# TAMUparametric/PPOPT

Hardware: NVIDIA B200
Metric: candidate active sets/sec (higher is better)
Workload: dtype f64

## Files before the change

### include/ppgpu.h

```cpp
#ifndef PPGPU_H
#define PPGPU_H

#include <stddef.h>
#include <stdint.h>

#ifdef __cplusplus
extern "C" {
#endif

typedef struct ppgpu_program ppgpu_program;
typedef void* ppgpu_stream;

typedef struct {
    int32_t n;
    int32_t t;
    int32_t m;
    int32_t q;
    int32_t n_eq;
    int32_t is_qp;
} ppgpu_dims;

typedef struct {
    int32_t words;
    int32_t n_ineq;
    int32_t region_rows;
    int32_t use_gram;
    int32_t max_depth;
    int32_t sm_count;
    int32_t lp_columns;
    int32_t reserved;
} ppgpu_info;

#define PPGPU_NUM_COUNTERS 24

const char* ppgpu_last_error(void);
int ppgpu_version(void);

int ppgpu_program_create(const ppgpu_dims* dims, const double* h_A, const double* h_b, const double* h_F,
                         const double* h_A_t, const double* h_b_t, const double* h_Q, const double* h_c,
                         const double* h_H, int device, ppgpu_program** out);
int ppgpu_program_destroy(ppgpu_program* prog);
int ppgpu_program_info(const ppgpu_program* prog, ppgpu_info* out);

#define PPGPU_OPT_K2W_MIN 0
int ppgpu_set_option(ppgpu_program* prog, int32_t option, int64_t value);

int ppgpu_root_level(ppgpu_program* prog, uint64_t* d_masks, int64_t* h_count, ppgpu_stream stream);

int ppgpu_level_eval(ppgpu_program* prog, const uint64_t* d_masks, int64_t n, int32_t k_act, uint8_t* d_status,
                     int32_t stages, ppgpu_stream stream);

#define PPGPU_WITNESS_SLOTS 2
int ppgpu_level_eval_w(ppgpu_program* prog, const uint64_t* d_masks, int64_t n, int32_t k_act, uint8_t* d_status,
                       int32_t stages, uint64_t* d_witness, const uint64_t* d_parent_feas, int64_t parent_nf,
                       const void* d_parent_ws, const uint64_t* d_parent_wit, ppgpu_stream stream);

size_t ppgpu_scan_workspace_bytes(int64_t n);
size_t ppgpu_select_workspace_bytes(int64_t n);
int ppgpu_level_select(ppgpu_program* prog, const uint8_t* d_status, int64_t n, uint8_t bits, uint8_t value,
                       int64_t* d_idx_out, int64_t* h_count, void* d_ws, size_t ws_bytes, ppgpu_stream stream);

int ppgpu_regions_emit(ppgpu_program* prog, const uint64_t* d_masks, const int64_t* d_sel, int64_t n_sel,
                       int32_t k_act, double* d_laws, double* d_rows, int32_t* d_flags, double* d_info,
                       uint8_t* d_status, ppgpu_stream stream);

int ppgpu_children_count(ppgpu_program* prog, const uint64_t* d_masks, const int64_t* d_feas_idx, int64_t nf,
                         int32_t k_act, uint64_t* d_feas_masks, uint64_t* d_survive, int64_t* d_offsets,
                         int64_t* h_total, void* d_ws, size_t ws_bytes, ppgpu_stream stream);
int ppgpu_children_prepare(ppgpu_program* prog, const uint64_t* d_masks, const int64_t* d_feas_idx, int64_t nf,
                           uint64_t* d_feas_masks, void* d_ws, size_t ws_bytes, ppgpu_stream stream);
int ppgpu_children_count_range(ppgpu_program* prog, const uint64_t* d_feas_masks, int64_t nf, int32_t k_act,
                               uint64_t* d_survive, int64_t* d_counts, int64_t p_lo, int64_t p_hi, void* d_ws,
                               size_t ws_bytes, ppgpu_stream stream);
int ppgpu_children_scan(ppgpu_program* prog, int64_t* d_counts_to_offsets, int64_t nf, int64_t* h_total, void* d_ws,
                        size_t ws_bytes, ppgpu_stream stream);
int ppgpu_children_write(ppgpu_program* prog, const uint64_t* d_feas_masks, const uint64_t* d_survive,
                         const int64_t* d_offsets, int64_t nf, uint64_t* d_children, ppgpu_stream stream);
// ... 42 lines not shown
```

### ppopt_b200/_lib.py

```python
import ctypes
import os

_HERE = os.path.dirname(os.path.abspath(__file__))
LIB_PATH = os.path.join(_HERE, 'libppgpu.so')

NUM_COUNTERS = 24
NUM_FAMILIES = 10
FAMILY_NAMES = ('k1_rank', 'k2_feas_lp', 'k34_kkt_cheb', 'k5_emit', 'k6_count', 'k6_write', 'select', 'k2a_relax', 'k2w_walk', 'inherit')
COUNTER_NAMES = ('k1_candidates', 'k2_lps', 'k2_pivots', 'k2_work', 'k4_lps', 'k4_pivots', 'k4_work', 'k5_lps',
                 'k5_pivots', 'k5_work', 'numeric', 'border', 'k6_lookups', 'k2a_tried', 'k2a_certified', 'k2a_steps', 'k2a_work',
                 'k2w_certified', 'k2w_pivots', 'k2w_work', 'k2w_giveup', 'inherited', 'inherit_lookups')

ST_RANK, ST_FEAS, ST_OPT, ST_REGION, ST_BORDER, ST_NUMERIC, ST_THIN = 1, 2, 4, 8, 16, 32, 64
OPT_K2W_MIN = 0
TREE_OPT_INHERIT = 0
WITNESS_SLOTS = 2


class Dims(ctypes.Structure):
    _fields_ = [(k, ctypes.c_int32) for k in ('n', 't', 'm', 'q', 'n_eq', 'is_qp')]


class Info(ctypes.Structure):
    _fields_ = [(k, ctypes.c_int32) for k in
                ('words', 'n_ineq', 'region_rows', 'use_gram', 'max_depth', 'sm_count', 'lp_columns', 'reserved')]


_vp, _i32, _i64, _u8, _sz = ctypes.c_void_p, ctypes.c_int32, ctypes.c_int64, ctypes.c_uint8, ctypes.c_size_t
SYMBOLS = {
    'ppgpu_last_error': (ctypes.c_char_p, []),
    'ppgpu_version': (ctypes.c_int, []),
    'ppgpu_program_create': (ctypes.c_int, [ctypes.POINTER(Dims)] + [_vp] * 8 + [ctypes.c_int, ctypes.POINTER(_vp)]),
    'ppgpu_program_destroy': (ctypes.c_int, [_vp]),
    'ppgpu_program_info': (ctypes.c_int, [_vp, ctypes.POINTER(Info)]),
    'ppgpu_set_option': (ctypes.c_int, [_vp, _i32, _i64]),
    'ppgpu_root_level': (ctypes.c_int, [_vp, _vp, ctypes.POINTER(_i64), _vp]),
    'ppgpu_level_eval': (ctypes.c_int, [_vp, _vp, _i64, _i32, _vp, _i32, _vp]),
    'ppgpu_level_eval_w': (ctypes.c_int, [_vp, _vp, _i64, _i32, _vp, _i32, _vp, _vp, _i64, _vp, _vp, _vp]),
    'ppgpu_scan_workspace_bytes': (_sz, [_i64]),
    'ppgpu_select_workspace_bytes': (_sz, [_i64]),
    'ppgpu_level_select': (ctypes.c_int, [_vp, _vp, _i64, _u8, _u8, _vp, ctypes.POINTER(_i64), _vp, _sz, _vp]),
    'ppgpu_regions_emit': (ctypes.c_int, [_vp, _vp, _vp, _i64, _i32, _vp, _vp, _vp, _vp, _vp, _vp]),
    'ppgpu_children_count': (ctypes.c_int, [_vp, _vp, _vp, _i64, _i32, _vp, _vp, _vp, ctypes.POINTER(_i64), _vp, _sz, _vp]),
    'ppgpu_children_prepare': (ctypes.c_int, [_vp, _vp, _vp, _i64, _vp, _vp, _sz, _vp]),
    'ppgpu_children_count_range': (ctypes.c_int, [_vp, _vp, _i64, _i32, _vp, _vp, _i64, _i64, _vp, _sz, _vp]),
    'ppgpu_children_scan': (ctypes.c_int, [_vp, _vp, _i64, ctypes.POINTER(_i64), _vp, _sz, _vp]),
    'ppgpu_children_write': (ctypes.c_int, [_vp, _vp, _vp, _vp, _i64, _vp, _vp]),
# ... 41 lines not shown
```

### ppopt_b200/csrc/api.cu

```cuda
#include <cstdio>
#include <cstdlib>
#include <cstring>
#include <mutex>
#include <string>
#include <vector>

#include "../../include/ppgpu.h"
#include "common.cuh"
#include "host_math.hpp"
#include "launch.h"

using namespace ppgpu;

static thread_local std::string g_err;

struct ppgpu_program {
    ReducedProgram host;
    DevProgram dev;
    int device = 0;
    int sm_count = 0;
    std::vector<void*> allocs;
    unsigned long long* d_counters = nullptr;
    unsigned long long* d_queue = nullptr;
    int queue_slot = 0;
    long long launches = 0;
    bool profiling = false;
    struct Span { int family; cudaEvent_t a, b; };
    std::vector<Span> spans;
    std::vector<cudaEvent_t> event_pool;
    long long warm_cap = 0;
    double* d_warm_resid = nullptr;
    long long* d_warm_idx = nullptr;
    unsigned long long* d_warm_count = nullptr;
    int* d_k2w_order = nullptr;
    size_t k2w_order_cap = 0;
    long long k2w_min = 100000;
    double prof_ms[PPGPU_NUM_FAMILIES] = {0};
    long long prof_launches[PPGPU_NUM_FAMILIES] = {0};
};

struct ProfScope {
    ppgpu_program* p; cudaStream_t st; int family; cudaEvent_t a = nullptr, b = nullptr;
    static cudaEvent_t get(ppgpu_program* p) {
        if (!p->event_pool.empty()) { cudaEvent_t e = p->event_pool.back(); p->event_pool.pop_back(); return e; }
        cudaEvent_t e; cudaEventCreate(&e); return e;
    }
    ProfScope(ppgpu_program* p_, cudaStream_t st_, int fam) : p(p_), st(st_), family(fam) {
        if (p->profiling) { a = get(p); b = get(p); cudaEventRecord(a, st); }
    }
    ~ProfScope() {
        if (a) { cudaEventRecord(b, st); p->spans.push_back({family, a, b}); }
    }
};

static const int QUEUE_SLOTS = 64;
extern "C" { static void warm_release(ppgpu_program* p); }

static int fail(const char* where, cudaError_t e) {
    g_err = std::string(where) + ": " + cudaGetErrorString(e);
    return -1;
}
static int fail_msg(const std::string& m) { g_err = m; return -2; }

template <class T>
static cudaError_t upload(ppgpu_program* p, const std::vector<T>& v, const T** out) {
    void* d = nullptr;
    const size_t bytes = v.size() * sizeof(T) + 1024;
    cudaError_t e = cudaMalloc(&d, bytes);
    if (e != cudaSuccess) return e;
// ... 67 lines not shown
            (e = upload(p, R.X0t, &D.X0t)) != cudaSuccess || (e = upload(p, R.Q2, &D.Q2)) != cudaSuccess) {
            ppgpu_program_destroy(p);
            return fail("upload LP start dictionary", e);
        }
    }
    void* dc = nullptr;
    if ((e = cudaMalloc(&dc, (CNT_COUNT + QUEUE_SLOTS) * sizeof(unsigned long long))) != cudaSuccess) {
        ppgpu_program_destroy(p);
        return fail("cudaMalloc counters", e);
    }
    p->allocs.push_back(dc);
    cudaMemset(dc, 0, (CNT_COUNT + QUEUE_SLOTS) * sizeof(unsigned long long));
    p->d_counters = (unsigned long long*)dc;
    p->d_queue = p->d_counters + CNT_COUNT;
    *out = p;
    return 0;
}

int ppgpu_program_destroy(ppgpu_program* p) {
    if (!p) return 0;
    for (void* d : p->allocs) cudaFree(d);
    if (p->d_k2w_order) cudaFree(p->d_k2w_order);
    warm_release(p);
    for (auto& s : p->spans) { cudaEventDestroy(s.a); cudaEventDestroy(s.b); }
    for (cudaEvent_t e : p->event_pool) cudaEventDestroy(e);
    delete p;
    return 0;
}

int ppgpu_set_option(ppgpu_program* p, int32_t option, int64_t value) {
    if (!p) return fail_msg("null argument");
    switch (option) {
        case PPGPU_OPT_K2W_MIN: p->k2w_min = value; return 0;
        default: return fail_msg("unknown option");
    }
}

int ppgpu_program_info(const ppgpu_program* p, ppgpu_info* o) {
    if (!p || !o) return fail_msg("null argument");
    const ReducedProgram& R = p->host;
    o->words = R.W; o->n_ineq = R.mi; o->region_rows = R.R0; o->use_gram = R.use_gram;
    o->max_depth = (R.n > R.t ? R.n : R.t) - R.ne;
    o->sm_count = p->sm_count;
    o->lp_columns = k2_pad_columns(R.nfree + 2);
    o->reserved = R.wk_ok;
    return 0;
}

int ppgpu_root_level(ppgpu_program* p, uint64_t* d_masks, int64_t* h_count, ppgpu_stream stream) {
    if (!p || !h_count) return fail_msg("null argument");
    long long cnt = 0;
    cudaError_t e = root_level(p->dev, d_masks, &cnt, (cudaStream_t)stream);
    if (e != cudaSuccess) return fail("root_level", e);
    p->launches += cnt > 0;
    *h_count = cnt;
    return 0;
}

static long long level_chunk() {
    static const long long c = getenv("PPGPU_CHUNK") ? atoll(getenv("PPGPU_CHUNK")) : (1ll << 22);
    return c < 1024 ? 1024 : c;
}
static long long walk_chunk() {
    static const long long c = getenv("PPGPU_WALK_CHUNK") ? atoll(getenv("PPGPU_WALK_CHUNK")) : (1ll << 27);
    return c < 1024 ? 1024 : c;
}
// ... 58 lines not shown
    cudaError_t e;
    if (stages & 1) {
        ProfScope ps(p, st, 0);
        const long long piece = 1ll << 22;
        for (long long off = 0; off < n; off += piece) {
            const long long nn = n - off < piece ? n - off : piece;
            e = launch_k1(p->dev, d_masks + (size_t)off * p->dev.W, nn, k_act, d_status + off, p->d_counters, p->sm_count, st);
            if (e != cudaSuccess) return fail("K1 rank", e);
            if (k_act >= 1 && k_act <= 8) p->launches++;
            p->launches++;
            if (k_act >= 2 && k_act <= p->dev.np) p->launches++;
        }
    }
    if ((stages & 2) && !(stages & 8) && wio.parent_feas && wio.parent_wit && wio.parent_ws && wio.parent_nf > 0) {
        ProfScope ps(p, st, 9);
        e = launch_inherit(p->dev, d_masks, n, d_status, wio.out, wio.parent_feas, wio.parent_nf, wio.parent_ws,
                           wio.parent_wit, p->d_counters, st);
        if (e != cudaSuccess) return fail("witness inheritance", e);
        p->launches++;
    }
    static const int warm_on = getenv("PPGPU_WARM") ? atoi(getenv("PPGPU_WARM")) : 1;
    p->dev.warm_count = nullptr; p->dev.warm_resid = nullptr; p->dev.warm_idx = nullptr; p->dev.warm_cap = 0;
    if ((stages & 2) && !(stages & 8) && k_act >= 1 && p->k2w_min >= 0 && n >= p->k2w_min) {
        ProfScope ps(p, st, 8);
        bool handled = false;
        const size_t want = k2w_order_scratch_ints(walk_chunk());
        if (want > p->k2w_order_cap) {
            if ((e = cudaStreamSynchronize(st)) != cudaSuccess) return fail("K2w order scratch", e);
            if (p->d_k2w_order) cudaFree(p->d_k2w_order);
            p->d_k2w_order = nullptr; p->k2w_order_cap = 0;
            if ((e = cudaMalloc((void**)&p->d_k2w_order, want * sizeof(int))) != cudaSuccess) return fail("K2w order scratch", e);
            p->k2w_order_cap = want;
        }
        e = launch_k2w(p->dev, d_masks, n, k_act, d_status, next_queue(p, st), p->d_counters, p->sm_count, st, &handled, wio.out, p->d_k2w_order);
        if (e != cudaSuccess) return fail("K2w vertex walk", e);
        if (handled) p->launches += (n > 128ll * 8 * p->sm_count) ? 4 : 1;
    }
    if ((stages & 2) && !(stages & 8)) {
        ProfScope ps(p, st, 7);
        static const int iters = getenv("PPGPU_K2A_ITERS") ? atoi(getenv("PPGPU_K2A_ITERS")) : 96;
        if (iters > 0 && k_act >= 0) {
            if (warm_on) {
                const bool walked = k_act >= 1 && p->dev.wk_ok && p->k2w_min >= 0 && n >= p->k2w_min;
                const long long cap = n < 4096 ? n : 4096 + n / (walked ? 64 : 8);
                if ((e = ensure_warm(p, cap, st)) != cudaSuccess) return fail("warm-start buffers", e);
                p->dev.warm_count = p->d_warm_count; p->dev.warm_resid = p->d_warm_resid;
                p->dev.warm_idx = p->d_warm_idx; p->dev.warm_cap = cap;
                cudaMemsetAsync(p->d_warm_count, 0, sizeof(unsigned long long), st);
            }
            e = launch_k2a(p->dev, d_masks, n, k_act, d_status, next_queue(p, st), p->d_counters, iters,
                           p->sm_count, st);
            if (e != cudaSuccess) return fail("K2a relaxation", e);
            p->launches++;
        }
    }
    if (stages & 2) {
        ProfScope ps(p, st, 1);
        e = launch_k2(p->dev, d_masks, n, d_status, next_queue(p, st), p->d_counters, p->sm_count, st);
        if (e != cudaSuccess) return fail("K2 feasibility", e);
        p->launches++;
        if (p->dev.warm_count) {
            if ((e = launch_clear_bits(d_status, n, PPG_ST_PRE, st)) != cudaSuccess) return fail("status clean-up", e);
            p->launches++;
        }
    }
    if (stages & 4) {
        ProfScope ps(p, st, 2);
// ... 412 lines not shown
```

### ppopt_b200/csrc/common.cuh

```cuda
#pragma once
#include <cuda_runtime.h>
#include <stdint.h>

#include "tolerances.h"

namespace ppgpu {

struct DevProgram {
    int n, t, m, q, ne, is_qp;
    int mi, np, W, R0, nfree, use_gram;
    int dc0;
    const double* At;
    const double* C1;
    const double* T0;
    const double* Gam;
    const double* G;
    const double* V;
    const double* th_lo; const double* th_hi;
    const double* A; const double* b; const double* F;
    const double* A_t; const double* b_t;
    const double* Q; const double* c; const double* H;
    const double* Xp;
    const double* K;
    const double* Pm;
    double* warm_resid;
    long long* warm_idx;
    unsigned long long* warm_count;
    long long warm_cap;
    int wk_ok, wk_nb, wk_ld;
    const double* wk_D0;
    const int* wk_bvar;
    const int* wk_nvar;
    int lp_ok, lp_ld;
    const double* lp_D0;
    const int* lp_bvar;
    const int* lp_nvar;
    const double* lp_obj;
    const double* X0t;
    const double* Q2;
};

enum Counter {
    CNT_K1_CAND = 0,
    CNT_K2_LPS, CNT_K2_PIVOTS, CNT_K2_WORK,
    CNT_K4_LPS, CNT_K4_PIVOTS, CNT_K4_WORK,
    CNT_K5_LPS, CNT_K5_PIVOTS, CNT_K5_WORK,
    CNT_NUMERIC, CNT_BORDER, CNT_K6_LOOKUPS,
    CNT_K2A_TRIED, CNT_K2A_CERTIFIED, CNT_K2A_STEPS,
    CNT_K2A_WORK,
    CNT_K2W_CERTIFIED, CNT_K2W_PIVOTS, CNT_K2W_WORK,
    CNT_K2W_GIVEUP,
    CNT_INHERITED, CNT_INHERIT_LOOKUPS,
    CNT_COUNT = 24
};

__device__ __forceinline__ bool mask_test(const uint64_t* m, int i) { return (m[i >> 6] >> (i & 63)) & 1ull; }

__device__ __forceinline__ int mask_popc(const uint64_t* m, int W) {
    int c = 0;
    for (int w = 0; w < W; ++w) c += __popcll(m[w]);
    return c;
}

__device__ __forceinline__ int mask_nth(const uint64_t* m, int W, int j) {
    for (int w = 0; w < W; ++w) {
        const uint64_t x = m[w];
        const int c = __popcll(x);
        if (j < c) {
            const unsigned lo = (unsigned)x, hi = (unsigned)(x >> 32);
            const int cl = __popc(lo);
            if (j < cl) return w * 64 + (int)__fns(lo, 0, j + 1);
            return w * 64 + 32 + (int)__fns(hi, 0, j - cl + 1);
        }
        j -= c;
    }
    return -1;
}

__device__ __forceinline__ int mask_rank(const uint64_t* m, int i) {
    int c = 0;
    const int w = i >> 6;
    for (int k = 0; k < w; ++k) c += __popcll(m[k]);
    const int b = i & 63;
    if (b) c += __popcll(m[w] & ((1ull << b) - 1ull));
    return c;
}
// ... 20 lines not shown
```

### ppopt_b200/csrc/k2w_walk.cu

```cuda
#include "common.cuh"
#include "launch.h"
#include "lp_core.cuh"

#include <cstdlib>

namespace ppgpu {

constexpr int K2W_MAXFIX = 30;
constexpr int K2W_DRIVE_CAP = 400;
constexpr int K2W_RESET = 3000;
constexpr double K2W_PIV_MIN = 1e-7;
constexpr double K2W_NEG_OK = 1e-8;

struct K2wCtx {
    double* D;
    double* prow;
    int* bvar;
    int* nvar;
    int* where;
    uint64_t* orig;
    uint64_t* todo;
    int* rowstart;
    uint64_t* nbm;
    int* fixrow;
    uint64_t* witness;
    int nb, nf, ld, lds, R0, W4, Wm;
};

__device__ __forceinline__ int k2w_top_bit(const uint64_t* m, int W, int* second) {
    int hi1 = -1, hi2 = -1;
    for (int w = W - 1; w >= 0 && hi2 < 0; --w) {
        uint64_t x = m[w];
        while (x && hi2 < 0) {
            const int t = w * 64 + 63 - __clzll((long long)x);
            x &= ~(1ull << (t & 63));
            if (hi1 < 0) hi1 = t; else hi2 = t;
        }
    }
    *second = hi2;
    return hi1;
}

__device__ __forceinline__ int k2w_nth(const uint64_t (&m)[4], int j) {
#pragma unroll
    for (int w = 0; w < 4; ++w) {
// ... 10 lines not shown

__device__ __forceinline__ double k2w_rcp(double x) {
    double r;
    asm("rcp.approx.ftz.f64 %0, %1;" : "=d"(r) : "d"(x));
    r = r * fma(-x, r, 2.0);
    return r * fma(-x, r, 2.0);
}

__device__ __forceinline__ void k2w_swap_labels(const K2wCtx& c, int l, int j) {
    const int rl = c.bvar[l], rn = c.nvar[j];
    c.bvar[l] = rn; c.nvar[j] = rl;
    c.where[rn] = l; c.where[rl] = ~j;
    c.nbm[rn >> 6] &= ~(1ull << (rn & 63));
    c.nbm[rl >> 6] |= 1ull << (rl & 63);
}

__device__ __forceinline__ void k2w_reload_labels(const DevProgram& P, const K2wCtx& c, int lane) {
    for (int w = lane; w < c.W4; w += 32) c.nbm[w] = 0ull;
    __syncwarp();
    for (int i = lane; i < c.nb; i += 32) { const int v = __ldg(P.wk_bvar + i); c.bvar[i] = v; c.where[v] = i; }
    for (int j = lane; j < c.nf; j += 32) {
        const int v = __ldg(P.wk_nvar + j);
        c.nvar[j] = v; c.where[v] = ~j;
        atomicOr(reinterpret_cast<unsigned long long*>(c.nbm + (v >> 6)), 1ull << (v & 63));
    }
    __syncwarp();
}

template <int RPL_, int LD_ = 0>
struct K2wSmemDict {
    static constexpr int RPL = RPL_;
    static constexpr bool IN_SMEM = true;
    static constexpr int SMEM_ROW0 = 0;
    __device__ __forceinline__ void reload(const DevProgram& P, const K2wCtx& c, int lane) {
        for (int e = lane; e < c.nb * c.ld; e += 32) {
            const int r = e / c.ld, k = e - r * c.ld;
            c.D[(size_t)r * c.lds + k] = __ldg(P.wk_D0 + e);
        }
        k2w_reload_labels(P, c, lane);
    }
    __device__ __forceinline__ void target_scan(const K2wCtx& c, int wi, uint64_t fm, int lane, double& bi, double& wbest, int& j) {
        const int lds = LD_ > 0 ? LD_ : c.lds;
        const double* Di = c.D + (size_t)wi * lds;
        bi = Di[0];
        const bool degen = bi <= 1e-11;
        double best = 0.0; int bj = 0x7fffffff;
        for (int jj = lane; jj < c.nf; jj += 32) {
            if ((fm >> jj) & 1ull) continue;
            double x = Di[1 + jj];
            if (degen) x = fabs(x);
            if (x > best) { best = x; bj = jj; }
        }
        wbest = warp_max_nonneg(best);
        j = __reduce_min_sync(PPG_FULL, best == wbest ? bj : 0x7fffffff);
    }
    __device__ __forceinline__ void column(const K2wCtx& c, int j, int lane, double (&col)[RPL], double (&beta)[RPL]) {
#pragma unroll
        for (int rr = 0; rr < RPL; ++rr) {
            const int r = lane + 32 * rr;
            const int lds = LD_ > 0 ? LD_ : c.lds;
            col[rr] = r < c.nb ? c.D[(size_t)r * lds + 1 + j] : 0.0;
            beta[rr] = r < c.nb ? c.D[(size_t)r * lds] : 0.0;
        }
    }
    __device__ __forceinline__ bool pivot(const K2wCtx& c, int l, int j, int lane) {
        const int cj = 1 + j, lds = LD_ > 0 ? LD_ : c.lds, ld = LD_ > 0 ? LD_ : c.ld, nb = c.nb;
// ... 52 lines not shown
#pragma unroll
                    for (int g = 0; g < G; ++g) x[rr][g] = (k0 + g < ld) ? Dr[rr][k0 + g] : 0.0;
#pragma unroll
                for (int rr = 0; rr < RPL; ++rr)
#pragma unroll
                    for (int g = 0; g < G; ++g) x[rr][g] = fma(-colr[rr], qk[g], x[rr][g]);
#pragma unroll
                for (int rr = 0; rr < RPL; ++rr)
                    if (colr[rr] != 0.0) {
#pragma unroll
                        for (int g = 0; g < G; ++g)
                            if (k0 + g < ld) Dr[rr][k0 + g] = x[rr][g];
                    }
            }
        }
        bool ok = okb;
#pragma unroll
        for (int rr = 0; rr < RPL; ++rr) {
            const int r = lane + 32 * rr;
            if (r < nb && r != l) {
                if (colr[rr] != 0.0) Dr[rr][cj] = -colr[rr] * inv;
                if constexpr (LD_ == 0) ok = ok && Dr[rr][0] >= -K2W_NEG_OK;
            }
        }
        __syncwarp();
        for (int k = lane; k < ld; k += 32) Dl[k] = (k == cj) ? inv : q[k];
        if (lane == 0) k2w_swap_labels(c, l, j);
        ok = __all_sync(PPG_FULL, ok);
        __syncwarp();
        return ok;
    }
};

template <int RPL_, int LD>
struct K2wHybridDict {
    static constexpr int RPL = RPL_;
    static constexpr bool IN_SMEM = true;
    static constexpr int SMEM_ROW0 = 32;
    double T0[LD];
    __device__ __forceinline__ void reload(const DevProgram& P, const K2wCtx& c, int lane) {
#pragma unroll
        for (int k = 0; k < LD; ++k) T0[k] = lane < c.nb ? __ldg(P.wk_D0 + (size_t)lane * LD + k) : 0.0;
        for (int e = lane + 32 * LD; e < c.nb * LD; e += 32) c.D[e - 32 * LD] = __ldg(P.wk_D0 + e);
        k2w_reload_labels(P, c, lane);
    }
    __device__ __forceinline__ void target_scan(const K2wCtx& c, int wi, uint64_t fm, int lane, double& bi, double& wbest, int& j) {
        if (wi < 32) {
            const double b0 = T0[0];
            const bool degen = b0 <= 1e-11;
            double best = 0.0; int bj = 0x7fffffff;
#pragma unroll
            for (int k = 1; k < LD; ++k) {
                double x = T0[k];
                if (degen) x = fabs(x);
                if (!((fm >> (k - 1)) & 1ull) && x > best) { best = x; bj = k - 1; }
            }
            bi = shfl_d(b0, wi);
            wbest = shfl_d(best, wi);
            j = __shfl_sync(PPG_FULL, bj, wi);
        } else {
            const double* Di = c.D + (size_t)(wi - 32) * LD;
            bi = Di[0];
            const bool degen = bi <= 1e-11;
            double best = 0.0; int bj = 0x7fffffff;
            for (int jj = lane; jj < c.nf; jj += 32) {
                if ((fm >> jj) & 1ull) continue;
                double x = Di[1 + jj];
                if (degen) x = fabs(x);
                if (x > best) { best = x; bj = jj; }
            }
            wbest = warp_max_nonneg(best);
// ... 67 lines not shown
                for (int rr = 1; rr < RPL; ++rr) {
                    const int r = lane + 32 * rr;
                    okb = okb && (r >= nb || r == l || x[rr][0] >= -K2W_NEG_OK);
                }
            }
#pragma unroll
            for (int rr = 1; rr < RPL; ++rr)
                if (colr[rr] != 0.0) {
#pragma unroll
                    for (int g = 0; g < GN; ++g) Dr[rr][k0 + g] = x[rr][g];
                }
        });
        reg_set<LD>(T0, cj, own ? inv : -colr[0] * inv);
#pragma unroll
        for (int rr = 1; rr < RPL; ++rr) {
            const int r = lane + 32 * rr;
            if (r < nb && r != l && colr[rr] != 0.0) Dr[rr][cj] = -colr[rr] * inv;
        }
        __syncwarp();
        if (!l_in_regs)
            for (int k = lane; k < LD; k += 32) Dl[k] = (k == cj) ? inv : q[k];
        if (lane == 0) k2w_swap_labels(c, l, j);
        const bool ok = __all_sync(PPG_FULL, okb);
        __syncwarp();
        return ok;
    }
};

template <int RPL_, int DC>
struct K2wRegDict {
    static constexpr int RPL = RPL_;
    static constexpr bool IN_SMEM = false;
    static constexpr int SMEM_ROW0 = 0;
    double T[RPL][DC];
    __device__ __forceinline__ void reload(const DevProgram& P, const K2wCtx& c, int lane) {
        static_for<RPL>([&](auto RR) {
            constexpr int rr = decltype(RR)::value;
            const int r = lane + 32 * rr;
#pragma unroll
            for (int k = 0; k < DC; ++k) T[rr][k] = r < c.nb ? __ldg(P.wk_D0 + (size_t)r * DC + k) : 0.0;
        });
        k2w_reload_labels(P, c, lane);
    }
    __device__ __forceinline__ void target_scan(const K2wCtx& c, int wi, uint64_t fm, int lane, double& bi, double& wbest, int& j) {
        const int slot = wi >> 5, owner = wi & 31;
        double b0 = 0.0, best = 0.0; int bj = 0x7fffffff;
        static_for<RPL>([&](auto RR) {
            constexpr int rr = decltype(RR)::value;
            if (rr == slot) {
                b0 = T[rr][0];
                const bool degen = b0 <= 1e-11;
#pragma unroll
                for (int k = 1; k < DC; ++k) {
                    double x = T[rr][k];
                    if (degen) x = fabs(x);
                    if (!((fm >> (k - 1)) & 1ull) && x > best) { best = x; bj = k - 1; }
                }
            }
        });
        bi = shfl_d(b0, owner);
        wbest = shfl_d(best, owner);
        j = __shfl_sync(PPG_FULL, bj, owner);
    }
    __device__ __forceinline__ void column(const K2wCtx& c, int j, int lane, double (&col)[RPL], double (&beta)[RPL]) {
        static_for<RPL>([&](auto RR) {
            constexpr int rr = decltype(RR)::value;
// ... 155 lines not shown
                    *cw &= ~rb;
                    k2w_certify(c, status, seg_base, y, r);
                    ++got;
                }
            }
        }
        __syncwarp();
    }
    return got;
}

template <class Dict>
__host__ __device__ constexpr size_t k2w_dict_smem_bytes(int nb, int lds) {
    if constexpr (!Dict::IN_SMEM) return 0;
    else return (size_t)(nb > Dict::SMEM_ROW0 ? nb - Dict::SMEM_ROW0 : 0) * lds * 8;
}

template <class Dict>
__global__ void __launch_bounds__(256, 1)
k2w_walk_kernel(DevProgram P, const uint64_t* __restrict__ masks, long long n, int k_act, uint8_t* __restrict__ status,
                unsigned long long* __restrict__ queue, unsigned long long* __restrict__ counters, int chunk,
                int walker_bytes, int lds, int W4, int group_items, int split_len, uint64_t* __restrict__ witness,
                const int* __restrict__ order, long long items) {
    extern __shared__ unsigned char k2w_smem[];
    const int warp = threadIdx.x >> 5, lane = threadIdx.x & 31;
    constexpr int RPL = Dict::RPL;
    Dict dict;
    K2wCtx c;
    c.nb = P.wk_nb; c.nf = P.nfree; c.ld = P.wk_ld; c.lds = lds; c.R0 = P.R0; c.W4 = W4;
    c.witness = witness; c.Wm = P.W;
    {
        unsigned char* base = k2w_smem + (size_t)warp * walker_bytes;
        c.D = reinterpret_cast<double*>(base); base += k2w_dict_smem_bytes<Dict>(c.nb, lds);
        c.prow = reinterpret_cast<double*>(base); base += (size_t)lds * 8;
        c.orig = reinterpret_cast<uint64_t*>(base); base += (size_t)c.R0 * W4 * 8;
        c.todo = reinterpret_cast<uint64_t*>(base); base += (size_t)c.R0 * W4 * 8;
        c.nbm = reinterpret_cast<uint64_t*>(base); base += (size_t)W4 * 8;
        c.bvar = reinterpret_cast<int*>(base); base += (size_t)c.nb * 4;
        c.nvar = reinterpret_cast<int*>(base); base += (size_t)c.nf * 4;
        c.where = reinterpret_cast<int*>(base); base += (size_t)c.R0 * 4;
        c.rowstart = reinterpret_cast<int*>(base); base += (size_t)c.R0 * 4;
        c.fixrow = reinterpret_cast<int*>(base);
    }
    const int W = P.W, R0 = P.R0, nb = c.nb, nf = c.nf;
    const int p = k_act >= 2 ? k_act - 2 : 0;
    unsigned long long n_piv = 0, n_give = 0;
    int n_cert = 0;
    auto split = [&](long long q, uint64_t (&pf)[4], int& a, int& b) {
#pragma unroll
        for (int w = 0; w < 4; ++w) pf[w] = w < W ? masks[q * W + w] : 0ull;
        b = k2w_top_bit(pf, W, &a);
        if (k_act < 2) a = b;
        pf[b >> 6] &= ~(1ull << (b & 63));
        if (k_act >= 2) pf[a >> 6] &= ~(1ull << (a & 63));
    };
    auto seg_end = [&](long long from, long long limit, const uint64_t (&pf0)[4], int a_ref) -> long long {
        for (long long q0 = from; q0 < limit; q0 += 32) {
            const long long q = q0 + lane;
            bool same = true;
            if (q < limit) {
                uint64_t m[4]; int a1, b1;
                split(q, m, a1, b1);
                same = m[0] == pf0[0] && m[1] == pf0[1] && m[2] == pf0[2] && m[3] == pf0[3] && (a_ref < 0 || a1 == a_ref);
            }
            const unsigned diff = __ballot_sync(PPG_FULL, !same);
            if (diff) return q0 + __ffs((int)diff) - 1;
        }
        return limit;
    };
    for (;;) {
        unsigned long long v = 0;
        if (lane == 0) {
            v = atomicAdd(queue, 1ull);
            if (v < (unsigned long long)items && order) v = (unsigned long long)order[v];
        }
        const long long item = (long long)__shfl_sync(PPG_FULL, v, 0);
        if (item >= items) break;
        const long long c0 = item * chunk;
        const long long c1 = (c0 + chunk < n) ? c0 + chunk : n;
// ... 23 lines not shown
            int any = 0;
            for (long long q0 = i; q0 < s1; q0 += 32) {
                const long long q = q0 + lane;
                int a1 = -1, b1 = -1;
                bool open = false;
                if (q < s1) {
                    uint64_t m[4];
                    split(q, m, a1, b1);
                    const uint8_t sb = status[q];
                    open = (sb & PPG_ST_RANK) && !(sb & PPG_ST_FEAS);
                    atomicOr(reinterpret_cast<unsigned long long*>(c.orig + (size_t)a1 * W4 + (b1 >> 6)), 1ull << (b1 & 63));
                    if ((sb & PPG_ST_RANK) && a1 != b1)
                        atomicOr(reinterpret_cast<unsigned long long*>(c.orig + (size_t)b1 * W4 + (a1 >> 6)), 1ull << (a1 & 63));
                    if (open) {
                        atomicOr(reinterpret_cast<unsigned long long*>(c.todo + (size_t)a1 * W4 + (b1 >> 6)), 1ull << (b1 & 63));
                        if (a1 != b1) atomicOr(reinterpret_cast<unsigned long long*>(c.todo + (size_t)b1 * W4 + (a1 >> 6)), 1ull << (a1 & 63));
                    }
                }
                int aprev = __shfl_up_sync(PPG_FULL, a1, 1);
                if (lane == 0) {
                    aprev = -1;
                    if (q0 > i) { uint64_t m[4]; int b2; split(q0 - 1, m, aprev, b2); }
                }
                if (q < s1 && a1 != aprev) c.rowstart[a1] = (int)(q - i);
                any |= __any_sync(PPG_FULL, open) ? 1 : 0;
            }
            __syncwarp();
            if (!any) { i = s1; continue; }
            int stage = 0, f = 0, a = -1, t = -1;
            uint64_t pmask = 0ull, fm = 0ull;
            bool restart = (npiv > K2W_RESET) || !vertex_ok;
            for (;;) {
                if (restart) {
                    dict.reload(P, c, lane);
                    n_piv += npiv; npiv = 0; nfixed = 0; vertex_ok = true; restart = false;
                    stage = 0; f = 0; a = -1;
                }
                if (stage == 0) {
                    if (f == 0) {
                        int keep = 0;
                        for (; keep < nfixed && keep < p; ++keep)
                            if (c.fixrow[keep] != k2w_nth(pf0, keep)) break;
                        nfixed = keep; f = keep;
                        pmask = 0ull;
                        for (int g = 0; g < nfixed; ++g) pmask |= 1ull << (~c.where[c.fixrow[g]]);
                    }
                    if (f < p) {
                        t = k2w_nth(pf0, f); fm = pmask;
                    } else {
                        n_cert += k2w_mark_all(c, status, i, lane);
                        __syncwarp();
                        if (c.witness && k_act >= 2) k2w_revisit_all(c, status, i, lane);
                        stage = 1; a = -1;
                    }
                }
                if (stage == 1) {
                    int na = -1;
                    for (int x = a + 1; x < R0 && na < 0; ++x)
                        for (int w = 0; w < W4; ++w)
                            if (c.todo[(size_t)x * W4 + w] & k2w_ge_mask(x, w)) { na = x; break; }
                    if (na < 0) break;
                    a = na; t = a; fm = pmask;
                    if (npiv > K2W_RESET) { restart = true; continue; }
                }
                if (stage == 2) {
                    int b = -1;
// ... 57 lines not shown
                    break;
                }
                if (stage == 0) {
                    if (!reached) { ++n_give; break; }
                    if (lane == 0) c.fixrow[f] = t;
                    __syncwarp();
                    pmask |= 1ull << (~c.where[t]);
                    nfixed = ++f;
                } else if (stage == 1) {
                    if (!reached) {
                        ++n_give;
                        if (lane == 0) for (int w = 0; w < W4; ++w) c.todo[(size_t)a * W4 + w] &= ~k2w_ge_mask(a, w);
                        __syncwarp();
                    } else if (k_act >= 2) {
                        fm = pmask | (1ull << (~c.where[a]));
                        stage = 2;
                    }
                } else {
                    if (lane == 0) c.todo[(size_t)a * W4 + (t >> 6)] &= ~(1ull << (t & 63));
                    __syncwarp();
                    if (!reached) ++n_give;
                }
            }
            i = s1;
        }
        n_piv += npiv;
    }
    n_cert = __reduce_add_sync(PPG_FULL, n_cert);
    if (lane == 0 && (n_piv || n_cert)) {
        atomicAdd(&counters[CNT_K2W_CERTIFIED], (unsigned long long)n_cert);
        atomicAdd(&counters[CNT_K2W_PIVOTS], n_piv);
        atomicAdd(&counters[CNT_K2W_WORK], n_piv * (unsigned long long)(c.nb * c.ld));
        atomicAdd(&counters[CNT_K2W_GIVEUP], n_give);
    }
}

constexpr int K2W_COST_BUCKETS = 1025;

__global__ void __launch_bounds__(256) k2w_item_cost_kernel(const uint8_t* __restrict__ status, long long n, int chunk, long long items,
                                                            int* __restrict__ cost, int* __restrict__ hist) {
    const int lane = threadIdx.x & 31;
    const long long item = ((long long)blockIdx.x * blockDim.x + threadIdx.x) >> 5;
    if (item >= items) return;
    const long long c0 = item * chunk, c1 = (c0 + chunk < n) ? c0 + chunk : n;
    int cnt = 0;
    for (long long q = c0 + lane; q < c1; q += 32) {
        const uint8_t sb = status[q];
        cnt += ((sb & PPG_ST_RANK) && !(sb & PPG_ST_FEAS)) ? 1 : 0;
    }
    cnt = __reduce_add_sync(PPG_FULL, cnt);
    if (cnt > K2W_COST_BUCKETS - 1) cnt = K2W_COST_BUCKETS - 1;
    if (lane == 0) { cost[item] = cnt; atomicAdd(&hist[K2W_COST_BUCKETS - 1 - cnt], 1); }
}

__global__ void __launch_bounds__(1024) k2w_item_scan_kernel(int* __restrict__ hist) {
    __shared__ int sh[K2W_COST_BUCKETS + 1];
    for (int i = threadIdx.x; i < K2W_COST_BUCKETS; i += blockDim.x) sh[i] = hist[i];
    __syncthreads();
    if (threadIdx.x == 0) {
        int run = 0;
        for (int i = 0; i < K2W_COST_BUCKETS; ++i) { const int c = sh[i]; sh[i] = run; run += c; }
    }
    __syncthreads();
    for (int i = threadIdx.x; i < K2W_COST_BUCKETS; i += blockDim.x) hist[i] = sh[i];
}

__global__ void __launch_bounds__(256) k2w_item_scatter_kernel(const int* __restrict__ cost, long long items, int* __restrict__ offs,
                                                               int* __restrict__ order) {
    const long long item = (long long)blockIdx.x * blockDim.x + threadIdx.x;
    if (item >= items) return;
    const int pos = atomicAdd(&offs[K2W_COST_BUCKETS - 1 - cost[item]], 1);
    order[pos] = (int)item;
}

size_t k2w_order_scratch_ints(long long n) { return (size_t)(2 * (n / 128 + 2) + K2W_COST_BUCKETS); }

static cudaError_t k2w_order_items(const uint8_t* status, long long n, int chunk, long long items, int* scratch, cudaStream_t st,
                                   const int** order_out) {
    int* cost = scratch;
    int* order = scratch + items;
    int* hist = scratch + 2 * items;
    cudaError_t e = cudaMemsetAsync(hist, 0, K2W_COST_BUCKETS * sizeof(int), st);
    if (e != cudaSuccess) return e;
    k2w_item_cost_kernel<<<(unsigned)((items * 32 + 255) / 256), 256, 0, st>>>(status, n, chunk, items, cost, hist);
    k2w_item_scan_kernel<<<1, 1024, 0, st>>>(hist);
    k2w_item_scatter_kernel<<<(unsigned)((items + 255) / 256), 256, 0, st>>>(cost, items, hist, order);
    *order_out = order;
    return cudaGetLastError();
}

#define K2W_COMMA ,
template <class Dict>
static cudaError_t launch_k2w_t(const DevProgram& P, const uint64_t* masks, long long n, int k_act, uint8_t* status,
                                unsigned long long* queue, unsigned long long* counters, int sm_count, cudaStream_t st,
                                bool* handled, uint64_t* witness, int* order_scratch) {
    const int nb = P.wk_nb, ld = P.wk_ld, lds = ld | 1, W4 = (P.R0 + 63) / 64;
    size_t wb = k2w_dict_smem_bytes<Dict>(nb, lds) + (size_t)lds * 8 + (size_t)2 * P.R0 * W4 * 8 + (size_t)W4 * 8 +
                (size_t)(nb + P.nfree + 2 * P.R0 + K2W_MAXFIX + 2) * 4;
    wb = (wb + 15) & ~(size_t)15;
    auto kern = k2w_walk_kernel<Dict>;
    cudaFuncAttributes fa;
    cudaError_t e = cudaFuncGetAttributes(&fa, kern);
    if (e != cudaSuccess) return e;
    int wpc = (int)((size_t)(226 * 1024) / wb);
    const int by_regs = 65536 / (32 * (fa.numRegs > 0 ? fa.numRegs : 255));
    if (wpc > by_regs) wpc = by_regs;
    if (wpc > 8) wpc = 8;
    if (wpc < 1) return cudaSuccess;
    const size_t smem = wb * wpc;
    e = allow_max_smem(kern);
    if (e != cudaSuccess) return e;
    const long long walkers = (long long)sm_count * wpc;
    static const long long chunk_env = getenv("PPGPU_K2W_ITEM") ? atoll(getenv("PPGPU_K2W_ITEM")) : 0;
    long long chunk = chunk_env > 0 ? chunk_env : n / (walkers * 12);
    if (chunk > 1024) chunk = 1024;
    if (chunk < 128) chunk = 128;
    long long grid = (n + chunk * wpc - 1) / (chunk * wpc);
    if (grid > sm_count) grid = sm_count;
    if (grid < 1) grid = 1;
    static const int groups_env = getenv("PPGPU_K2W_GROUPS") ? atoi(getenv("PPGPU_K2W_GROUPS")) : -1;
    static const int split_len = getenv("PPGPU_K2W_SPLIT") ? atoi(getenv("PPGPU_K2W_SPLIT")) : 2048;
    const int group_items = groups_env >= 0 ? groups_env : (n / walkers < 16384 ? 1 : 0);
    const long long items = (n + chunk - 1) / chunk;
    const int* order = nullptr;
    static const int lpt_on = getenv("PPGPU_K2W_LPT") ? atoi(getenv("PPGPU_K2W_LPT")) : 1;
    if (lpt_on && order_scratch && items > walkers && items < (1ll << 30)) {
        if ((e = k2w_order_items(status, n, (int)chunk, items, order_scratch, st, &order)) != cudaSuccess) return e;
    }
    kern<<<(unsigned)grid, 32 * wpc, smem, st>>>(P, masks, n, k_act, status, queue, counters, (int)chunk, (int)wb, lds, W4,
                                                 group_items, split_len, witness, order, items);
    *handled = true;
    return cudaGetLastError();
}

cudaError_t launch_k2w(const DevProgram& P, const uint64_t* masks, long long n, int k_act, uint8_t* status,
                       unsigned long long* queue, unsigned long long* counters, int sm_count, cudaStream_t st, bool* handled,
                       uint64_t* witness, int* order_scratch) {
    *handled = false;
    static const int on = getenv("PPGPU_K2W") ? atoi(getenv("PPGPU_K2W")) : 1;
    static const int regs_on = getenv("PPGPU_K2W_REG") ? atoi(getenv("PPGPU_K2W_REG")) : 0;
    if (!on || !P.wk_ok || k_act < 1 || k_act - 2 > K2W_MAXFIX || P.W > 4 || P.nfree > 64) return cudaSuccess;
    const int rpl = (P.wk_nb + 31) / 32;
#define K2W_GO(D) return launch_k2w_t<D>(P, masks, n, k_act, status, queue, counters, sm_count, st, handled, witness, order_scratch)
    if (regs_on && rpl == 3 && P.wk_ld == 37) K2W_GO(K2wRegDict<3 K2W_COMMA 37>);
    static const int hybrid_on = getenv("PPGPU_K2W_HYBRID") ? atoi(getenv("PPGPU_K2W_HYBRID")) : 0;
    if (hybrid_on && rpl == 3 && P.wk_ld == 37) K2W_GO(K2wHybridDict<3 K2W_COMMA 37>);
    if (rpl == 3 && P.wk_ld == 37) K2W_GO(K2wSmemDict<3 K2W_COMMA 37>);
    switch (rpl) {
        case 1: K2W_GO(K2wSmemDict<1>);
        case 2: K2W_GO(K2wSmemDict<2>);
        case 3: K2W_GO(K2wSmemDict<3>);
        case 4: K2W_GO(K2wSmemDict<4>);
        case 5: K2W_GO(K2wSmemDict<5>);
        case 6: K2W_GO(K2wSmemDict<6>);
        case 7: K2W_GO(K2wSmemDict<7>);
        case 8: K2W_GO(K2wSmemDict<8>);
        default: return cudaSuccess;
    }
#undef K2W_GO
}

}
```

### ppopt_b200/csrc/launch.h

```cpp
#pragma once
#include <cuda_runtime.h>
#include <stdint.h>

#include "common.cuh"

namespace ppgpu {

template <class K>
inline cudaError_t allow_max_smem(K kern) {
    int dev = 0, lim = 0;
    cudaError_t e = cudaGetDevice(&dev);
    if (e == cudaSuccess) e = cudaDeviceGetAttribute(&lim, cudaDevAttrMaxSharedMemoryPerBlockOptin, dev);
    if (e != cudaSuccess) return e;
    cudaFuncAttributes fa;
    if ((e = cudaFuncGetAttributes(&fa, kern)) != cudaSuccess) return e;
    return cudaFuncSetAttribute(kern, cudaFuncAttributeMaxDynamicSharedMemorySize, lim - (int)fa.sharedSizeBytes);
}

template <class K>
inline cudaError_t fit_smem(K kern, size_t dyn) {
    cudaFuncAttributes fa;
    const cudaError_t e = cudaFuncGetAttributes(&fa, kern);
    if (e != cudaSuccess) return e;
    return fa.sharedSizeBytes + dyn > 48 * 1024 ? allow_max_smem(kern) : cudaSuccess;
}

int k2_pad_columns(int ncols_with_rhs);

cudaError_t launch_k1(const DevProgram& P, const uint64_t* masks, long long n, int k_act, uint8_t* status,
                      unsigned long long* counters, int sm_count, cudaStream_t st);
cudaError_t launch_k2(const DevProgram& P, const uint64_t* masks, long long n, uint8_t* status,
                      unsigned long long* queue, unsigned long long* counters, int sm_count, cudaStream_t st);
cudaError_t launch_k2a(const DevProgram& P, const uint64_t* masks, long long n, int k_act, uint8_t* status,
                       unsigned long long* queue, unsigned long long* counters, int max_iter, int sm_count, cudaStream_t st);
cudaError_t launch_k2a_prefix(const DevProgram& P, const uint64_t* masks, long long n, int k_act, uint8_t* status,
                              unsigned long long* queue, unsigned long long* counters, int max_iter, int sm_count,
                              cudaStream_t st, bool* handled);
cudaError_t launch_k2w(const DevProgram& P, const uint64_t* masks, long long n, int k_act, uint8_t* status,
                       unsigned long long* queue, unsigned long long* counters, int sm_count, cudaStream_t st, bool* handled,
                       uint64_t* witness, int* order_scratch);
size_t k2w_order_scratch_ints(long long n);
cudaError_t launch_inherit(const DevProgram& P, const uint64_t* masks, long long n, uint8_t* status, uint64_t* witness_out,
                           const uint64_t* parent_feas, long long parent_nf, const void* parent_ws, const uint64_t* parent_wit,
                           unsigned long long* counters, cudaStream_t st);
cudaError_t launch_k34(const DevProgram& P, const uint64_t* masks, long long n, int k_act, uint8_t* status,
                       unsigned long long* queue, unsigned long long* counters, int sm_count, cudaStream_t st);
cudaError_t launch_k34_compact(const DevProgram& P, const uint64_t* masks, long long n, int k_act, uint8_t* status,
                               unsigned long long* queue, unsigned long long* counters, int sm_count, cudaStream_t st,
                               int use_pre, bool* handled);
cudaError_t launch_mark_general(const DevProgram& P, long long n, int k_act, uint8_t* status, cudaStream_t st);

cudaError_t launch_k5(const DevProgram& P, const uint64_t* masks, const long long* idx, long long n_sel, int k_act,
                      double* laws, double* rows, int32_t* flags, double* info, uint8_t* status,
                      unsigned long long* queue, unsigned long long* counters, int sm_count, cudaStream_t st);
int k5_launches(int t);

size_t scan_workspace_bytes(long long n);
size_t select_workspace_bytes(long long n);
const long long* children_order_flag(const void* ws, long long nf);
cudaError_t select_indices(const uint8_t* status, long long n, uint8_t bits, uint8_t value, long long* idx_out,
                           long long* d_count, void* ws, size_t ws_bytes, cudaStream_t st);
cudaError_t root_level(const DevProgram& P, uint64_t* masks, long long* d_count, cudaStream_t st);
cudaError_t children_count(const DevProgram& P, const uint64_t* masks, const long long* feas_idx, long long nf,
                           int k_act, uint64_t* feas_masks, uint64_t* survive, long long* offsets, void* ws,
                           size_t ws_bytes, unsigned long long* counters, cudaStream_t st);
cudaError_t children_prepare(const DevProgram& P, const uint64_t* masks, const long long* feas_idx, long long nf,
                             uint64_t* feas_masks, void* ws, size_t ws_bytes, cudaStream_t st);
cudaError_t children_count_range(const DevProgram& P, const uint64_t* feas_masks, long long nf, int k_act, uint64_t* survive,
                                 long long* counts, long long p_lo, long long p_hi, void* ws, unsigned long long* counters,
                                 cudaStream_t st);
cudaError_t children_scan(long long* counts_to_offsets, long long nf, void* ws, cudaStream_t st);
cudaError_t children_write(const DevProgram& P, const uint64_t* feas_masks, const uint64_t* survive,
                           const long long* offsets, long long nf, uint64_t* children, cudaStream_t st);
// ... 36 lines not shown
```

Before: 369.8 million.

## Add deferred rank-K dictionary updates to K2w vertex walk

Adds a K2wDeferDict that holds up to K=2 pivot updates as low-rank factors (u vectors plus pivot rows) and applies them lazily when rows and columns are read, flushing the combined update to shared memory only every K pivots. The aim is fewer full passes over the shared-memory dictionary per pivot in the LD=37, RPL=3 case, which becomes the default path. The old smem dictionary is kept behind a new reference option, and counters are added for deferred work discarded at resets or give-ups. In exchange there is extra chain arithmetic per access, more registers, and possible numerical drift.

Result: faster. 396.4 million (median of 6 runs) (+7.2%).

```diff
diff --git a/include/ppgpu.h b/include/ppgpu.h
--- a/include/ppgpu.h
+++ b/include/ppgpu.h
@@ -31,7 +31,7 @@
     int32_t reserved;
 } ppgpu_info;
 
-#define PPGPU_NUM_COUNTERS 24
+#define PPGPU_NUM_COUNTERS 26
 
 const char* ppgpu_last_error(void);
 int ppgpu_version(void);
@@ -43,6 +43,7 @@
 int ppgpu_program_info(const ppgpu_program* prog, ppgpu_info* out);
 
 #define PPGPU_OPT_K2W_MIN 0
+#define PPGPU_OPT_K2W_REF 1
 int ppgpu_set_option(ppgpu_program* prog, int32_t option, int64_t value);
 
 int ppgpu_root_level(ppgpu_program* prog, uint64_t* d_masks, int64_t* h_count, ppgpu_stream stream);
diff --git a/ppopt_b200/_lib.py b/ppopt_b200/_lib.py
--- a/ppopt_b200/_lib.py
+++ b/ppopt_b200/_lib.py
@@ -4,15 +4,17 @@
 _HERE = os.path.dirname(os.path.abspath(__file__))
 LIB_PATH = os.path.join(_HERE, 'libppgpu.so')
 
-NUM_COUNTERS = 24
+NUM_COUNTERS = 26
 NUM_FAMILIES = 10
 FAMILY_NAMES = ('k1_rank', 'k2_feas_lp', 'k34_kkt_cheb', 'k5_emit', 'k6_count', 'k6_write', 'select', 'k2a_relax', 'k2w_walk', 'inherit')
 COUNTER_NAMES = ('k1_candidates', 'k2_lps', 'k2_pivots', 'k2_work', 'k4_lps', 'k4_pivots', 'k4_work', 'k5_lps',
                  'k5_pivots', 'k5_work', 'numeric', 'border', 'k6_lookups', 'k2a_tried', 'k2a_certified', 'k2a_steps', 'k2a_work',
-                 'k2w_certified', 'k2w_pivots', 'k2w_work', 'k2w_giveup', 'inherited', 'inherit_lookups')
+                 'k2w_certified', 'k2w_pivots', 'k2w_work', 'k2w_giveup', 'inherited', 'inherit_lookups',
+                 'k2w_drop_reset', 'k2w_drop_giveup')
 
 ST_RANK, ST_FEAS, ST_OPT, ST_REGION, ST_BORDER, ST_NUMERIC, ST_THIN = 1, 2, 4, 8, 16, 32, 64
 OPT_K2W_MIN = 0
+OPT_K2W_REF = 1
 TREE_OPT_INHERIT = 0
 WITNESS_SLOTS = 2
 
diff --git a/ppopt_b200/csrc/api.cu b/ppopt_b200/csrc/api.cu
--- a/ppopt_b200/csrc/api.cu
+++ b/ppopt_b200/csrc/api.cu
@@ -35,6 +35,7 @@
     int* d_k2w_order = nullptr;
     size_t k2w_order_cap = 0;
     long long k2w_min = 100000;
+    bool k2w_ref = false;
     double prof_ms[PPGPU_NUM_FAMILIES] = {0};
     long long prof_launches[PPGPU_NUM_FAMILIES] = {0};
 };
@@ -168,6 +169,7 @@
     if (!p) return fail_msg("null argument");
     switch (option) {
         case PPGPU_OPT_K2W_MIN: p->k2w_min = value; return 0;
+        case PPGPU_OPT_K2W_REF: p->k2w_ref = value != 0; return 0;
         default: return fail_msg("unknown option");
     }
 }
@@ -292,7 +294,8 @@
             if ((e = cudaMalloc((void**)&p->d_k2w_order, want * sizeof(int))) != cudaSuccess) return fail("K2w order scratch", e);
             p->k2w_order_cap = want;
         }
-        e = launch_k2w(p->dev, d_masks, n, k_act, d_status, next_queue(p, st), p->d_counters, p->sm_count, st, &handled, wio.out, p->d_k2w_order);
+        e = launch_k2w(p->dev, d_masks, n, k_act, d_status, next_queue(p, st), p->d_counters, p->sm_count, st, &handled, wio.out, p->d_k2w_order,
+                       p->k2w_ref);
         if (e != cudaSuccess) return fail("K2w vertex walk", e);
         if (handled) p->launches += (n > 128ll * 8 * p->sm_count) ? 4 : 1;
     }
diff --git a/ppopt_b200/csrc/common.cuh b/ppopt_b200/csrc/common.cuh
--- a/ppopt_b200/csrc/common.cuh
+++ b/ppopt_b200/csrc/common.cuh
@@ -51,7 +51,8 @@
     CNT_K2W_CERTIFIED, CNT_K2W_PIVOTS, CNT_K2W_WORK,
     CNT_K2W_GIVEUP,
     CNT_INHERITED, CNT_INHERIT_LOOKUPS,
-    CNT_COUNT = 24
+    CNT_K2W_DROP_RESET, CNT_K2W_DROP_GIVEUP,
+    CNT_COUNT = 26
 };
 
 __device__ __forceinline__ bool mask_test(const uint64_t* m, int i) { return (m[i >> 6] >> (i & 63)) & 1ull; }
diff --git a/ppopt_b200/csrc/k2w_walk.cu b/ppopt_b200/csrc/k2w_walk.cu
--- a/ppopt_b200/csrc/k2w_walk.cu
+++ b/ppopt_b200/csrc/k2w_walk.cu
@@ -11,6 +11,7 @@
 constexpr int K2W_RESET = 3000;
 constexpr double K2W_PIV_MIN = 1e-7;
 constexpr double K2W_NEG_OK = 1e-8;
+constexpr int K2W_DEFER = 2;
 
 struct K2wCtx {
     double* D;
@@ -87,6 +88,7 @@
     static constexpr int RPL = RPL_;
     static constexpr bool IN_SMEM = true;
     static constexpr int SMEM_ROW0 = 0;
+    static constexpr int PROWS = 1;
     __device__ __forceinline__ void reload(const DevProgram& P, const K2wCtx& c, int lane) {
         for (int e = lane; e < c.nb * c.ld; e += 32) {
             const int r = e / c.ld, k = e - r * c.ld;
@@ -205,11 +207,184 @@
     }
 };
 
+template <int RPL_, int LD, int K>
+struct K2wDeferDict {
+    static constexpr int RPL = RPL_;
+    static constexpr bool IN_SMEM = true;
+    static constexpr int SMEM_ROW0 = 0;
+    static constexpr int PROWS = K;
+    double u[K][RPL];
+    double beta[RPL];
+    int np;
+    static constexpr int TH = (LD - 1 + 31) / 32;
+    double trow[TH], ccol[RPL];
+    int trow_i, ccol_j;
+    template <int N>
+    __device__ __forceinline__ double from_row(const double (&v)[N], int slot, int owner) const {
+        double x = 0.0;
+#pragma unroll
+        for (int rr = 0; rr < N; ++rr) if (rr == slot) x = v[rr];
+        return shfl_d(x, owner);
+    }
+    __device__ __forceinline__ void row_u(int l, double (&ul)[K]) const {
+#pragma unroll
+        for (int m = 0; m < K; ++m) ul[m] = m < np ? from_row(u[m], l >> 5, l & 31) : 0.0;
+    }
+    __device__ __forceinline__ double chain(const K2wCtx& c, double x, const double (&um)[K], int k) const {
+#pragma unroll
+        for (int m = 0; m < K; ++m)
+            if (m < np) x = fma(-um[m], c.prow[m * LD + k], x);
+        return x;
+    }
+    __device__ __forceinline__ void reload(const DevProgram& P, const K2wCtx& c, int lane) {
+        for (int e = lane; e < c.nb * LD; e += 32) c.D[e] = __ldg(P.wk_D0 + e);
+#pragma unroll
+        for (int rr = 0; rr < RPL; ++rr) {
+            const int r = lane + 32 * rr;
+            beta[rr] = r < c.nb ? __ldg(P.wk_D0 + (size_t)r * LD) : 0.0;
+        }
+        np = 0;
+        trow_i = -1; ccol_j = -1;
+        k2w_reload_labels(P, c, lane);
+    }
+    __device__ __forceinline__ void target_scan(const K2wCtx& c, int wi, uint64_t fm, int lane, double& bi, double& wbest, int& j) {
+        double uw[K];
+        row_u(wi, uw);
+        bi = from_row(beta, wi >> 5, wi & 31);
+        const double* Di = c.D + (size_t)wi * LD;
+        const bool degen = bi <= 1e-11;
+        double best = 0.0; int bj = 0x7fffffff;
+#pragma unroll
+        for (int h = 0; h < TH; ++h) {
+            const int jj = lane + 32 * h;
+            if (1 + jj >= LD) continue;
+            trow[h] = chain(c, Di[1 + jj], uw, 1 + jj);
+            if (jj >= c.nf || ((fm >> jj) & 1ull)) continue;
+            const double x = degen ? fabs(trow[h]) : trow[h];
+            if (x > best) { best = x; bj = jj; }
+        }
+        trow_i = wi;
+        wbest = warp_max_nonneg(best);
+        j = __reduce_min_sync(PPG_FULL, best == wbest ? bj : 0x7fffffff);
+    }
+    __device__ __forceinline__ void cur_column(const K2wCtx& c, int cj, int lane, double (&col)[RPL]) const {
+#pragma unroll
+        for (int rr = 0; rr < RPL; ++rr) {
+            const int r = lane + 32 * rr;
+            double um[K];
+#pragma unroll
+            for (int m = 0; m < K; ++m) um[m] = u[m][rr];
+            col[rr] = r < c.nb ? chain(c, c.D[(size_t)r * LD + cj], um, cj) : 0.0;
+        }
+    }
+    __device__ __forceinline__ void column(const K2wCtx& c, int j, int lane, double (&col)[RPL], double (&beta_out)[RPL]) {
+        cur_column(c, 1 + j, lane, col);
+#pragma unroll
+        for (int rr = 0; rr < RPL; ++rr) { ccol[rr] = col[rr]; beta_out[rr] = beta[rr]; }
+        ccol_j = j;
+    }
+    __device__ __forceinline__ bool pivot(const K2wCtx& c, int l, int j, int lane) {
+        const int cj = 1 + j, nb = c.nb, slot = l >> 5, owner = l & 31;
+        double col[RPL];
+        if (ccol_j == j) {
+#pragma unroll
+            for (int rr = 0; rr < RPL; ++rr) col[rr] = ccol[rr];
+        } else {
+            cur_column(c, cj, lane, col);
+        }
+        const double inv = k2w_rcp(from_row(col, slot, owner));
+        double ul[K];
+        row_u(l, ul);
+        const double q0 = from_row(beta, slot, owner) * inv;
+        __syncwarp();
+        double* Dl = c.D + (size_t)l * LD;
+        double* pn = c.prow + np * LD;
+        if (lane == 0) pn[0] = q0;
+#pragma unroll
+        for (int h = 0; h < TH; ++h) {
+            const int k = 1 + lane + 32 * h;
+            if (k >= LD) continue;
+            const double x = trow_i == l ? trow[h] : chain(c, Dl[k], ul, k);
+            const double q = (k == cj) ? 0.0 : x * inv;
+            pn[k] = q;
+            Dl[k] = (k == cj) ? inv : q;
+        }
+        trow_i = -1; ccol_j = -1;
+        bool ok = true;
+#pragma unroll
+        for (int rr = 0; rr < RPL; ++rr) {
+            const int r = lane + 32 * rr;
+            if (r == l) {
+#pragma unroll
+                for (int m = 0; m < K; ++m) if (m < np) u[m][rr] = 0.0;
+            }
+            const double ur = (r < nb && r != l) ? col[rr] : 0.0;
+#pragma unroll
+            for (int m = 0; m < K; ++m) if (m == np) u[m][rr] = ur;
+            const double x = fma(-ur, q0, beta[rr]);
+            beta[rr] = r == l ? q0 : x;
+            ok = ok && (r >= nb || r == l || x >= -K2W_NEG_OK);
+            if (r < nb && r != l) c.D[(size_t)r * LD + cj] = -ur * inv;
+        }
+        __syncwarp();
+        if (lane < np) c.prow[lane * LD + cj] = 0.0;
+        if (lane == 0) k2w_swap_labels(c, l, j);
+        if (++np == K) {
+            __syncwarp();
+            flush(c, lane);
+        }
+        ok = __all_sync(PPG_FULL, ok);
+        __syncwarp();
+        return ok;
+    }
+    __device__ __forceinline__ void flush(const K2wCtx& c, int lane) {
+        constexpr int G = 6;
+        double* Dr[RPL];
+        bool st[RPL];
+#pragma unroll
+        for (int rr = 0; rr < RPL; ++rr) {
+            const int r = lane + 32 * rr;
+            Dr[rr] = c.D + (size_t)(r < c.nb ? r : 0) * LD;
+            st[rr] = false;
+#pragma unroll
+            for (int m = 0; m < K; ++m) st[rr] = st[rr] || u[m][rr] != 0.0;
+        }
+        const double* __restrict__ p = c.prow;
+        static_for<(LD - 1 + G - 1) / G>([&](auto KK) {
+            constexpr int k0 = 1 + decltype(KK)::value * G;
+            constexpr int GN = (LD - k0) < G ? (LD - k0) : G;
+            double x[RPL][GN];
+#pragma unroll
+            for (int rr = 0; rr < RPL; ++rr)
+#pragma unroll
+                for (int g = 0; g < GN; ++g) x[rr][g] = Dr[rr][k0 + g];
+#pragma unroll
+            for (int m = 0; m < K; ++m) {
+                double pk[GN];
+#pragma unroll
+                for (int g = 0; g < GN; ++g) pk[g] = p[m * LD + k0 + g];
+#pragma unroll
+                for (int rr = 0; rr < RPL; ++rr)
+#pragma unroll
+                    for (int g = 0; g < GN; ++g) x[rr][g] = fma(-u[m][rr], pk[g], x[rr][g]);
+            }
+#pragma unroll
+            for (int rr = 0; rr < RPL; ++rr)
+                if (st[rr]) {
+#pragma unroll
+                    for (int g = 0; g < GN; ++g) Dr[rr][k0 + g] = x[rr][g];
+                }
+        });
+        np = 0;
+    }
+};
+
 template <int RPL_, int LD>
 struct K2wHybridDict {
     static constexpr int RPL = RPL_;
     static constexpr bool IN_SMEM = true;
     static constexpr int SMEM_ROW0 = 32;
+    static constexpr int PROWS = 1;
     double T0[LD];
     __device__ __forceinline__ void reload(const DevProgram& P, const K2wCtx& c, int lane) {
 #pragma unroll
@@ -343,6 +518,7 @@
     static constexpr int RPL = RPL_;
     static constexpr bool IN_SMEM = false;
     static constexpr int SMEM_ROW0 = 0;
+    static constexpr int PROWS = 1;
     double T[RPL][DC];
     __device__ __forceinline__ void reload(const DevProgram& P, const K2wCtx& c, int lane) {
         static_for<RPL>([&](auto RR) {
@@ -564,7 +740,7 @@
     {
         unsigned char* base = k2w_smem + (size_t)warp * walker_bytes;
         c.D = reinterpret_cast<double*>(base); base += k2w_dict_smem_bytes<Dict>(c.nb, lds);
-        c.prow = reinterpret_cast<double*>(base); base += (size_t)lds * 8;
+        c.prow = reinterpret_cast<double*>(base); base += (size_t)Dict::PROWS * lds * 8;
         c.orig = reinterpret_cast<uint64_t*>(base); base += (size_t)c.R0 * W4 * 8;
         c.todo = reinterpret_cast<uint64_t*>(base); base += (size_t)c.R0 * W4 * 8;
         c.nbm = reinterpret_cast<uint64_t*>(base); base += (size_t)W4 * 8;
@@ -576,7 +752,7 @@
     }
     const int W = P.W, R0 = P.R0, nb = c.nb, nf = c.nf;
     const int p = k_act >= 2 ? k_act - 2 : 0;
-    unsigned long long n_piv = 0, n_give = 0;
+    unsigned long long n_piv = 0, n_give = 0, n_drop_reset = 0, n_drop_give = 0;
     int n_cert = 0;
     auto split = [&](long long q, uint64_t (&pf)[4], int& a, int& b) {
 #pragma unroll
@@ -666,6 +842,7 @@
             bool restart = (npiv > K2W_RESET) || !vertex_ok;
             for (;;) {
                 if (restart) {
+                    if (npiv % Dict::PROWS) ++(vertex_ok ? n_drop_reset : n_drop_give);
                     dict.reload(P, c, lane);
                     n_piv += npiv; npiv = 0; nfixed = 0; vertex_ok = true; restart = false;
                     stage = 0; f = 0; a = -1;
@@ -789,6 +966,8 @@
         atomicAdd(&counters[CNT_K2W_PIVOTS], n_piv);
         atomicAdd(&counters[CNT_K2W_WORK], n_piv * (unsigned long long)(c.nb * c.ld));
         atomicAdd(&counters[CNT_K2W_GIVEUP], n_give);
+        if (n_drop_reset) atomicAdd(&counters[CNT_K2W_DROP_RESET], n_drop_reset);
+        if (n_drop_give) atomicAdd(&counters[CNT_K2W_DROP_GIVEUP], n_drop_give);
     }
 }
 
@@ -852,7 +1031,7 @@
                                 unsigned long long* queue, unsigned long long* counters, int sm_count, cudaStream_t st,
                                 bool* handled, uint64_t* witness, int* order_scratch) {
     const int nb = P.wk_nb, ld = P.wk_ld, lds = ld | 1, W4 = (P.R0 + 63) / 64;
-    size_t wb = k2w_dict_smem_bytes<Dict>(nb, lds) + (size_t)lds * 8 + (size_t)2 * P.R0 * W4 * 8 + (size_t)W4 * 8 +
+    size_t wb = k2w_dict_smem_bytes<Dict>(nb, lds) + (size_t)Dict::PROWS * lds * 8 + (size_t)2 * P.R0 * W4 * 8 + (size_t)W4 * 8 +
                 (size_t)(nb + P.nfree + 2 * P.R0 + K2W_MAXFIX + 2) * 4;
     wb = (wb + 15) & ~(size_t)15;
     auto kern = k2w_walk_kernel<Dict>;
@@ -892,7 +1071,7 @@
 
 cudaError_t launch_k2w(const DevProgram& P, const uint64_t* masks, long long n, int k_act, uint8_t* status,
                        unsigned long long* queue, unsigned long long* counters, int sm_count, cudaStream_t st, bool* handled,
-                       uint64_t* witness, int* order_scratch) {
+                       uint64_t* witness, int* order_scratch, bool reference) {
     *handled = false;
     static const int on = getenv("PPGPU_K2W") ? atoi(getenv("PPGPU_K2W")) : 1;
     static const int regs_on = getenv("PPGPU_K2W_REG") ? atoi(getenv("PPGPU_K2W_REG")) : 0;
@@ -902,7 +1081,8 @@
     if (regs_on && rpl == 3 && P.wk_ld == 37) K2W_GO(K2wRegDict<3 K2W_COMMA 37>);
     static const int hybrid_on = getenv("PPGPU_K2W_HYBRID") ? atoi(getenv("PPGPU_K2W_HYBRID")) : 0;
     if (hybrid_on && rpl == 3 && P.wk_ld == 37) K2W_GO(K2wHybridDict<3 K2W_COMMA 37>);
-    if (rpl == 3 && P.wk_ld == 37) K2W_GO(K2wSmemDict<3 K2W_COMMA 37>);
+    if (rpl == 3 && P.wk_ld == 37 && reference) K2W_GO(K2wSmemDict<3 K2W_COMMA 37>);
+    if (rpl == 3 && P.wk_ld == 37) K2W_GO(K2wDeferDict<3 K2W_COMMA 37 K2W_COMMA K2W_DEFER>);
     switch (rpl) {
         case 1: K2W_GO(K2wSmemDict<1>);
         case 2: K2W_GO(K2wSmemDict<2>);
diff --git a/ppopt_b200/csrc/launch.h b/ppopt_b200/csrc/launch.h
--- a/ppopt_b200/csrc/launch.h
+++ b/ppopt_b200/csrc/launch.h
@@ -38,7 +38,7 @@
                               cudaStream_t st, bool* handled);
 cudaError_t launch_k2w(const DevProgram& P, const uint64_t* masks, long long n, int k_act, uint8_t* status,
                        unsigned long long* queue, unsigned long long* counters, int sm_count, cudaStream_t st, bool* handled,
-                       uint64_t* witness, int* order_scratch);
+                       uint64_t* witness, int* order_scratch, bool reference);
 size_t k2w_order_scratch_ints(long long n);
 cudaError_t launch_inherit(const DevProgram& P, const uint64_t* masks, long long n, uint8_t* status, uint64_t* witness_out,
                            const uint64_t* parent_feas, long long parent_nf, const void* parent_ws, const uint64_t* parent_wit,
```
